# ooshyun/Speech-Enhancement-Pytorch

Measured on AMD Instinct MI355X. Metric: audio-sec/sec training, DCCRN 16kHz 2s bs32, higher is better.
Workload: dtype bf16; 1 GPU; DCCRN (kernel_num 16-32-64-128-256-256, complex LSTM 128, mask E) train step, 16 kHz 2-s clips, SI-SNR, Adam 3e-4, clip 5; per_gpu_batch=32, global_batch=32, samples_per_clip=32000, parallelism=dp1, launch=eager, inputs=resident in HBM

## Files before the change

### include/sehip.h

```cpp
#ifndef SEHIP_H
#define SEHIP_H
#include <stdint.h>

#ifdef __cplusplus
extern "C" {
#endif

const char* sehip_last_error(void);
const char* sehip_last_kernel(void);
int sehip_version(void);
int sehip_check_device(int device);

void* sehip_event_create(void);
int sehip_event_destroy(void* event);
int sehip_stream_depend(void* to_stream, void* from_stream, void* event);
int sehip_event_record(void* event, void* stream);
int sehip_stream_wait_event(void* stream, void* event);
void* sehip_stream_create(int priority_class);
int sehip_stream_destroy(void* stream);

int sehip_stft_frames(int n_samples, int win_len, int hop);
int sehip_stft_fwd(const float* wav , const float* window , int B, int N, int win_len, int hop,
                   int fft_len, float* spec , void* enc_in_bf16 , void* stream);
int sehip_istft_fwd(const float* spec, const float* mask , const float* window,
// ... 191 lines not shown
                           long rows, int Cr, float* gWrr, float* gWri, float* gWii, float* gBr, float* gBi, float* gslope,
                           float* bcoef , void* stream);
int sehip_cbn_bwd_finalize_n(const float* part, int nblk, const float* coef, const float* Wrr, const float* Wri, const float* Wii,
                             long rows, int Cr, float* gWrr, float* gWri, float* gWii, float* gBr, float* gBi, float* gslope,
                             float* bcoef , void* stream);
int sehip_cbn_bwd_fused(const void* dz, const void* dz2 , const void* y, const float* coef, const float* Wrr, const float* Wri,
                        const float* Wii, const float* slope, long rows, int Cr, int F, int Tst, int tfirst, float* rep, float* rep_next,
                        int nrep,
                        float* gWrr, float* gWri, float* gWii, float* gBr, float* gBi, float* gslope, void* dy, void* stream);
int sehip_cbn_bwd_reduce_fin(const void* dz, const void* dz2 , const void* y, const float* coef, const float* Wrr,
                             const float* Wri, const float* Wii, const float* slope, long rows, int Cr, int F, int Tst, int tfirst,
                             float* rep, int nrep, unsigned* ticket, float* gWrr, float* gWri, float* gWii, float* gBr, float* gBi,
                             float* gslope, float* bcoef , void* stream);
int sehip_cbn_bwd_apply(const void* dz, const void* dz2, const void* y, const float* coef, const float* bcoef,
                        const float* slope, long rows, int Cr, int F, int Tst, int tfirst, void* dy, void* stream);

long sehip_rbn_scratch_floats(long rows, int Cs);
int sehip_rbn_stats(const void* y, long rows, int Cs, int Cr, float* part, void* stream);
int sehip_rbn_finalize(const float* part, const float* w_re, const float* b_re, const float* w_im, const float* b_im, float* rm_re,
                       float* rv_re, float* rm_im, float* rv_im, long* nbt_re, long* nbt_im, long rows, int Cs, int Cr, float eps,
                       float momentum, int training, float* coef, void* stream);
int sehip_rbn_finalize_s(const float* part, const float* w_re, const float* b_re, const float* w_im, const float* b_im, float* rm_re,
                         float* rv_re, float* rm_im, float* rv_im, long* nbt_re, long* nbt_im, long rows, int Cs, int Cr, float eps,
                         float momentum, int training, const float* shift, float* coef, void* stream);
int sehip_rbn_apply(const void* y, const float* coef, long rows, int Cs, int Cr, void* z, void* stream);
int sehip_rbn_bwd_reduce(const void* dz, const void* y, const float* coef, long rows, int Cs, int Cr, float* part, void* stream);
int sehip_rbn_bwd_reduce_fin(const void* dz, const void* y, const float* coef, long rows, int Cs, int Cr, float* part, unsigned* ticket,
                             float* gw_re, float* gb_re, float* gw_im, float* gb_im, float* bcoef, void* stream);
int sehip_rbn_bwd_finalize(const float* part, const float* coef, long rows, int Cs, int Cr, float* gw_re, float* gb_re, float* gw_im,
                           float* gb_im, float* bcoef, void* stream);
// ... 213 lines not shown
```

### speech-enhancement-pytorch_amd/sehip/_lib.py

```python
import ctypes as C
import os

import torch

_HERE = os.path.dirname(os.path.abspath(__file__))
LIB_PATH = os.environ.get("SEHIP_LIB") or os.path.join(_HERE, "libsehip.so")


class SehipError(RuntimeError):
    pass


_lib = None

P = C.c_void_p
I = C.c_int
L = C.c_long
F = C.c_float
U = C.c_uint
D = C.c_double

_PROTOS = {
    "sehip_version": [],
    "sehip_check_device": [I],
# ... 79 lines not shown
    "sehip_unpack_grad_sums_perm": [P, P, P, L, P, P, I, P, P, P, P, P],
    "sehip_unpack_grad1": [P, P, L, P, P],
    "sehip_unpack_grad1_sums": [P, P, L, P, P, I, P, P, P, P, P],
    "sehip_unpack_grad_list_sums": [P, P, P, L, P, P, I, P, P, P],
    "sehip_unpack_grad_list": [P, P, P, L, P, P],
    "sehip_pack_bf16_runs": [P, P, P, L, P, P],
    "sehip_pack_bf16_runs_to": [P, P, P, P, L, P, P],
    "sehip_cbn_stats": [P, L, I, P, P],
    "sehip_cbn_finalize": [P, P, P, P, P, P, P, P, P, P, P, P, L, I, F, F, I, P, P],
    "sehip_cbn_finalize_n": [P, I, P, P, P, P, P, P, P, P, P, P, P, L, I, F, F, I, P, P],
    "sehip_cbn_apply": [P, P, P, L, I, P, P],
    "sehip_cbn_finalize_apply_n": [P, P, I, P, P, P, P, P, P, P, P, P, P, P, L, I, F, F, I, P, P, P, P],
    "sehip_cbn_bwd_reduce": [P, P, P, P, P, L, I, I, I, I, P, P],
    "sehip_cbn_bwd_finalize": [P, P, P, P, P, L, I, P, P, P, P, P, P, P, P],
    "sehip_cbn_bwd_apply": [P, P, P, P, P, P, L, I, I, I, I, P, P],
    "sehip_cbn_bwd_fused": [P, P, P, P, P, P, P, P, L, I, I, I, I, P, P, I, P, P, P, P, P, P, P, P],
    "sehip_cbn_bwd_reduce_fin": [P, P, P, P, P, P, P, P, L, I, I, I, I, P, I, P, P, P, P, P, P, P, P, P],
    "sehip_rbn_scratch_floats": [L, I],
    "sehip_rbn_stats": [P, L, I, I, P, P],
    "sehip_rbn_finalize": [P, P, P, P, P, P, P, P, P, P, P, L, I, I, F, F, I, P, P],
    "sehip_rbn_finalize_s": [P, P, P, P, P, P, P, P, P, P, P, L, I, I, F, F, I, P, P, P],
    "sehip_rbn_apply": [P, P, L, I, I, P, P],
    "sehip_rbn_bwd_reduce": [P, P, P, L, I, I, P, P],
    "sehip_rbn_bwd_reduce_fin": [P, P, P, L, I, I, P, P, P, P, P, P, P, P],
    "sehip_rbn_bwd_finalize": [P, P, L, I, I, P, P, P, P, P, P],
    "sehip_rbn_bwd_apply": [P, P, P, P, L, I, I, P, P],
    "sehip_dcunet_pack_input": [P, I, I, I, P, P],
    "sehip_dcunet_mask_fwd": [P, P, P, P, P, P, I, I, I, I, I, I, P, P, P],
    "sehip_dcunet_mask_bwd": [P, P, P, P, P, P, I, I, I, I, I, I, P, P, P],
    "sehip_dcunet_mask_fwd_bn": [P, P, P, P, P, P, P, I, I, I, I, I, I, P, P, P],
# ... 187 lines not shown
```

### speech-enhancement-pytorch_amd/sehip/csrc/cbn.hip

```cpp
#include <stdlib.h>
#include "common.h"

#define COEF_STRIDE 16


template <int CH> struct Raw;
template <> struct Raw<8> { typedef uint4 type; };
template <> struct Raw<4> { typedef uint2 type; };
template <int CH> struct Chunk { float v[CH]; };
__device__ __forceinline__ Chunk<8> unpack(uint4 u) {
    Chunk<8> c;
    c.v[0] = bf2f((bf16_raw)(u.x & 0xffff)); c.v[1] = bf2f((bf16_raw)(u.x >> 16));
    c.v[2] = bf2f((bf16_raw)(u.y & 0xffff)); c.v[3] = bf2f((bf16_raw)(u.y >> 16));
    c.v[4] = bf2f((bf16_raw)(u.z & 0xffff)); c.v[5] = bf2f((bf16_raw)(u.z >> 16));
    c.v[6] = bf2f((bf16_raw)(u.w & 0xffff)); c.v[7] = bf2f((bf16_raw)(u.w >> 16));
    return c;
}
__device__ __forceinline__ Chunk<4> unpack(uint2 u) {
    Chunk<4> c;
    c.v[0] = bf2f((bf16_raw)(u.x & 0xffff)); c.v[1] = bf2f((bf16_raw)(u.x >> 16));
    c.v[2] = bf2f((bf16_raw)(u.y & 0xffff)); c.v[3] = bf2f((bf16_raw)(u.y >> 16));
    return c;
}
__device__ __forceinline__ void pack_store(bf16_raw* p, const float (&v)[8]) {
// ... 138 lines not shown
        RVri[c] = rvri + momentum * (vri - rvri);
        RVii[c] = rvii + momentum * (vii * unb - rvii);
        if (c == 0 && nbt) nbt[0] += 1;
    } else {
        if (threadIdx.x != 0) return;
        mr = rmr; mi = rmi; vrr = rvrr; vri = rvri; vii = rvii;
    }
    float rec[15];
    cbn_fwd_record(mr, mi, vrr, vri, vii, eps, wrr, wri, wii, br_, bi_, rec);
    float* o = coef + (size_t)c * COEF_STRIDE;
#pragma unroll
    for (int i = 0; i < 15; ++i) o[i] = rec[i];
}

template <int CH>
__device__ __forceinline__ void stage_coef(const float* __restrict__ rec, int Cr, int nfield, float4* __restrict__ slot) {
    const int nq = Cr / CH;
    for (int i = threadIdx.x; i < Cr * nfield; i += 256) {
        const int c = i / nfield, f = i - c * nfield;
        slot[f * Cr + (c % CH) * nq + (c / CH)] = reinterpret_cast<const float4*>(rec)[c * (COEF_STRIDE / 4) + f];
    }
}

template <int U, int CH>
__global__ __launch_bounds__(256, 2) void cbn_apply_kernel(const bf16_raw* __restrict__ y, const float* __restrict__ coef,
                                                           const float* __restrict__ slope, long rows, int Cr,
                                                           bf16_raw* __restrict__ z) {
    typedef typename Raw<CH>::type raw_t;
    __shared__ float4 cl[2 * 256];
    const int nq = Cr / CH;
    const int C = 2 * Cr;
    const int q = threadIdx.x % nq, rl = threadIdx.x / nq, rpb = 256 / nq;
    const float a = slope[0];
    stage_coef<CH>(coef, Cr, 2, cl);
    __syncthreads();
// ... 140 lines not shown
    v.gi = *reinterpret_cast<const raw_t*>(dz + o + Cr);
    if (HAS2) {
        v.hr = *reinterpret_cast<const raw_t*>(dz2 + o);
        v.hi = *reinterpret_cast<const raw_t*>(dz2 + o + Cr);
    }
    return v;
}

struct CbnFin {
    const float *Wrr, *Wri, *Wii;
    float *gWrr, *gWri, *gWii, *gBr, *gBi, *gslope, *bcoef;
    unsigned* ticket;
};
__device__ __forceinline__ void cbn_bwd_record(float sdr, float sdi, float qrr, float qri, float qir, float qii, float urr, float uri,
                                               float uii, float vrr, float vri, float vii, float wrr, float wri, float wii, float n,
                                               float (&g5)[5], float (&o)[9], float real = 0.f);

template <int U, int CH, bool HAS2>
__global__ __launch_bounds__(256, 2) void cbn_bwd_reduce_kernel(const bf16_raw* __restrict__ dz, const bf16_raw* __restrict__ dz2,
                                                                const bf16_raw* __restrict__ y, const float* __restrict__ coef,
                                                                const float* __restrict__ slope, long rows, int Cr, int F,
                                                                int Tst, int tfirst, float* __restrict__ part, int nrep, const CbnFin fin) {
    __shared__ float lds[4 * 6 * 8 * 32];
    const int nq = Cr / CH;
    const int q = threadIdx.x % nq, rl = threadIdx.x / nq, rpb = 256 / nq;
    const int C = 2 * Cr;
    const float a = slope[0];
    float s[6][CH];
#pragma unroll
    for (int u = 0; u < 6; ++u)
#pragma unroll
        for (int j = 0; j < CH; ++j) s[u][j] = 0.f;
    float da = 0.f;
// ... 26 lines not shown
            s[0][j] += dr; s[1][j] += di;
            s[2][j] += dr * cr; s[3][j] += dr * ci; s[4][j] += di * cr; s[5][j] += di * ci;
        }
    };
    const long stride = (long)gridDim.x * rpb;
    long r = (long)blockIdx.x * rpb + rl;
    for (; r + (U - 1) * stride < rows; r += U * stride) {
        RowIn<CH, HAS2> v[U];
#pragma unroll
        for (int u = 0; u < U; ++u) v[u] = load_row<CH, HAS2>(y, dz, dz2, (r + u * stride) * C + q * CH, Cr);
#pragma unroll
        for (int u = 0; u < U; ++u) row(v[u], r + u * stride);
    }
    if (U > 1)
        for (; r < rows; r += stride) row(load_row<CH, HAS2>(y, dz, dz2, r * C + q * CH, Cr), r);
    block_partials<6, CH>(s, nq, Cr, part, 6 * Cr + 1, lds, nrep);
    da = wave_sum(da);
    __syncthreads();
    if ((threadIdx.x & 63) == 0) lds[threadIdx.x >> 6] = da;
    __syncthreads();
    if (threadIdx.x == 0) {
        const float t = lds[0] + lds[1] + lds[2] + lds[3];
        if (nrep > 0) atomicAdd(&part[(size_t)(blockIdx.x % nrep) * (6 * Cr + 1) + 6 * Cr], t);
        else part[(size_t)blockIdx.x * (6 * Cr + 1) + 6 * Cr] = t;
    }
    if (nrep <= 0 || fin.ticket == nullptr) return;
    asm volatile("s_waitcnt vmcnt(0)" ::: "memory");
    __syncthreads();
    __shared__ unsigned is_last;
    if (threadIdx.x == 0) {
        __builtin_amdgcn_fence(__ATOMIC_RELEASE, "agent");
        asm volatile("s_waitcnt vmcnt(0)" ::: "memory");
        is_last = __hip_atomic_fetch_add(fin.ticket, 1u, __ATOMIC_RELAXED, __HIP_MEMORY_SCOPE_AGENT) == gridDim.x - 1 ? 1u : 0u;
    }
    __syncthreads();
    if (!is_last) return;
    if (threadIdx.x == 0) {
        __builtin_amdgcn_fence(__ATOMIC_ACQUIRE, "agent");
        asm volatile("s_waitcnt vmcnt(0)" ::: "memory");
    }
    __syncthreads();
    const int st = 6 * Cr + 1;
    for (int c = threadIdx.x; c < Cr; c += 256) {
        const float* k = coef + (size_t)c * COEF_STRIDE;
        const float urr = k[8], uri = k[9], uii = k[10], vrr = k[11], vri = k[12], vii = k[13];
        const float wrr = fin.Wrr[c], wri = fin.Wri[c], wii = fin.Wii[c];
        double a6[6] = {0.0, 0.0, 0.0, 0.0, 0.0, 0.0};
        for (int r0 = 0; r0 < nrep; r0 += 8) {
            float v[8][6];
#pragma unroll
            for (int r = 0; r < 8; ++r)
#pragma unroll
                for (int kk = 0; kk < 6; ++kk) v[r][kk] = part[(size_t)(r0 + r < nrep ? r0 + r : 0) * st + kk * Cr + c];
#pragma unroll
            for (int r = 0; r < 8; ++r)
#pragma unroll
                for (int kk = 0; kk < 6; ++kk) a6[kk] += r0 + r < nrep ? (double)v[r][kk] : 0.0;
        }
        float g5[5], rec[9];
        cbn_bwd_record((float)a6[0], (float)a6[1], (float)a6[2], (float)a6[3], (float)a6[4], (float)a6[5], urr, uri, uii, vrr, vri, vii,
                       wrr, wri, wii, (float)rows, g5, rec, k[14]);
        fin.gWrr[c] = g5[0]; fin.gWri[c] = g5[1]; fin.gWii[c] = g5[2]; fin.gBr[c] = g5[3]; fin.gBi[c] = g5[4];
        float* o = fin.bcoef + (size_t)c * COEF_STRIDE;
#pragma unroll
        for (int i = 0; i < 9; ++i) o[i] = rec[i];
    }
    if (threadIdx.x == 255) {
        double ds = 0.0;
        for (int r = 0; r < nrep; ++r) ds += (double)part[(size_t)r * st + 6 * Cr];
        fin.gslope[0] = (float)ds;
    }
    __syncthreads();
    for (int i = threadIdx.x; i < nrep * st; i += 256) part[i] = 0.f;
    if (threadIdx.x == 0) __hip_atomic_store(fin.ticket, 0u, __ATOMIC_RELAXED, __HIP_MEMORY_SCOPE_AGENT);
}

__device__ __forceinline__ void cbn_bwd_record(float sdr, float sdi, float qrr, float qri, float qir, float qii, float urr, float uri,
                                               float uii, float vrr, float vri, float vii, float wrr, float wri, float wii, float n,
                                               float (&g5)[5], float (&o)[9], float real) {
    if (real != 0.f) wri = 0.f;
    const float prr = qrr * urr + qri * uri, pri = qrr * uri + qri * uii;
    const float pir = qir * urr + qii * uri, pii = qir * uri + qii * uii;
    g5[0] = prr; g5[1] = pri + pir; g5[2] = pii; g5[3] = sdr; g5[4] = sdi;
    const float hrr = wrr * qrr + wri * qir, hri = wrr * qri + wri * qii;
    const float hir = wri * qrr + wii * qir, hii = wri * qri + wii * qii;
    const float dUrr = hrr, dUri = hri + hir, dUii = hii;
    const float tau = vrr + vii;
    const float delta = vrr * vii - vri * vri;
    const float s = sqrtf(delta);
    const float t = sqrtf(tau + 2.f * s);
    const float rst = 1.f / (s * t);
    const float d_rst = dUrr * (s + vii) - dUri * vri + dUii * (s + vrr);
    float d_s = (dUrr + dUii) * rst;
    float d_vii = dUrr * rst, d_vrr = dUii * rst, d_vri = -dUri * rst;
    d_s += d_rst * (-rst / s);
    const float d_t = d_rst * (-rst / t);
    const float d_tau = d_t / (2.f * t);
    d_s += d_t / t;
    const float d_delta = d_s / (2.f * s);
    d_vrr += d_delta * vii + d_tau;
    d_vii += d_delta * vrr + d_tau;
    d_vri += d_delta * (-2.f * vri);
    const float arr = urr * wrr + uri * wri, ari = urr * wri + uri * wii;
    const float air = uri * wrr + uii * wri, aii = uri * wri + uii * wii;
    o[0] = arr; o[1] = ari; o[2] = air; o[3] = aii;
    o[4] = 2.f * d_vrr / n; o[5] = d_vri / n; o[6] = 2.f * d_vii / n;
    o[7] = -(arr * sdr + ari * sdi) / n;
    o[8] = -(air * sdr + aii * sdi) / n;
    if (real != 0.f) { o[5] = 0.f; g5[1] = 0.f; }
}

template <int MAXB>
__global__ void cbn_bwd_finalize_kernel(const float* __restrict__ part, int nblk, const float* __restrict__ coef,
                                        const float* __restrict__ Wrr, const float* __restrict__ Wri,
                                        const float* __restrict__ Wii, long rows, int Cr, float* __restrict__ gWrr,
                                        float* __restrict__ gWri, float* __restrict__ gWii, float* __restrict__ gBr,
                                        float* __restrict__ gBi, float* __restrict__ gslope, float* __restrict__ bcoef) {
    const int c = blockIdx.x;
    const int st = 6 * Cr + 1;
    if (c == Cr) {
        double ds[1];
        wave_reduce_partials<1, MAXB>(part, nblk, st, 6 * Cr, Cr, ds);
        if (threadIdx.x == 0) gslope[0] = (float)ds[0];
        return;
    }
    const float* k = coef + (size_t)c * COEF_STRIDE;
    const float urr = k[8], uri = k[9], uii = k[10], vrr = k[11], vri = k[12], vii = k[13];
    const float wrr = Wrr[c], wri = Wri[c], wii = Wii[c];
    double a[6];
    wave_reduce_partials<6, MAXB>(part, nblk, st, c, Cr, a);
    const float sdr = (float)a[0], sdi = (float)a[1], qrr = (float)a[2], qri = (float)a[3], qir = (float)a[4], qii = (float)a[5];
    if (threadIdx.x != 0) return;
    float g5[5], rec[9];
    cbn_bwd_record(sdr, sdi, qrr, qri, qir, qii, urr, uri, uii, vrr, vri, vii, wrr, wri, wii, (float)rows, g5, rec, k[14]);
    gWrr[c] = g5[0]; gWri[c] = g5[1]; gWii[c] = g5[2]; gBr[c] = g5[3]; gBi[c] = g5[4];
    float* o = bcoef + (size_t)c * COEF_STRIDE;
#pragma unroll
    for (int i = 0; i < 9; ++i) o[i] = rec[i];
}

template <int U, int CH, bool HAS2>
__global__ __launch_bounds__(256, 2) void cbn_bwd_apply_kernel(const bf16_raw* __restrict__ dz, const bf16_raw* __restrict__ dz2,
                                                               const bf16_raw* __restrict__ y, const float* __restrict__ coef,
                                                               const float* __restrict__ bcoef, const float* __restrict__ slope,
                                                               long rows, int Cr, int F, int Tst, int tfirst,
                                                               bf16_raw* __restrict__ dy) {
    __shared__ float4 cl[5 * 256];
    const int nq = Cr / CH;
    const int C = 2 * Cr;
    const int q = threadIdx.x % nq, rl = threadIdx.x / nq, rpb = 256 / nq;
    const float a = slope[0];
    stage_coef<CH>(coef, Cr, 2, cl);
    stage_coef<CH>(bcoef, Cr, 3, cl + 2 * Cr);
    __syncthreads();
    float4 zc[CH], mb[CH], A[CH], E[CH];
    float ki[CH];
#pragma unroll
    for (int j = 0; j < CH; ++j) {
        zc[j] = cl[j * nq + q];
        mb[j] = cl[Cr + j * nq + q];
        A[j] = cl[2 * Cr + j * nq + q];
        E[j] = cl[3 * Cr + j * nq + q];
        ki[j] = cl[4 * Cr + j * nq + q].x;
    }
    auto row = [&](const RowIn<CH, HAS2>& v, long r) {
        const bool dropped = tfirst > 0 && (int)(((unsigned)r / (unsigned)F) % (unsigned)Tst) < tfirst;
        const Chunk<CH> xr = unpack(v.yr), xi = unpack(v.yi);
        Chunk<CH> gr = unpack(v.gr), gi = unpack(v.gi);
        if (HAS2) {
            const Chunk<CH> hr = unpack(v.hr), hi = unpack(v.hi);
#pragma unroll
            for (int j = 0; j < CH; ++j) { gr.v[j] += hr.v[j]; gi.v[j] += hi.v[j]; }
        }
        float orr[CH], oii[CH];
#pragma unroll
        for (int j = 0; j < CH; ++j) {
            const float cr = xr.v[j] - mb[j].x, ci = xi.v[j] - mb[j].y;
            const float vr = zc[j].x * cr + zc[j].y * ci + mb[j].z;
            const float vi = zc[j].z * cr + zc[j].w * ci + mb[j].w;
            float dr = dropped ? 0.f : gr.v[j], di = dropped ? 0.f : gi.v[j];
            if (!(vr > 0.f)) dr *= a;
            if (!(vi > 0.f)) di *= a;
            orr[j] = A[j].x * dr + A[j].y * di + E[j].x * cr + E[j].y * ci + E[j].w;
            oii[j] = A[j].z * dr + A[j].w * di + E[j].y * cr + E[j].z * ci + ki[j];
        }
        pack_store(dy + r * C + q * CH, orr);
        pack_store(dy + r * C + Cr + q * CH, oii);
    };
    const long stride = (long)gridDim.x * rpb;
    long r = (long)blockIdx.x * rpb + rl;
    for (; r + (U - 1) * stride < rows; r += U * stride) {
        RowIn<CH, HAS2> v[U];
#pragma unroll
        for (int u = 0; u < U; ++u) v[u] = load_row<CH, HAS2>(y, dz, dz2, (r + u * stride) * C + q * CH, Cr);
#pragma unroll
        for (int u = 0; u < U; ++u) row(v[u], r + u * stride);
    }
    if (U > 1)
        for (; r < rows; r += stride) row(load_row<CH, HAS2>(y, dz, dz2, r * C + q * CH, Cr), r);
}

template <int U, int CH, bool HAS2>
__global__ __launch_bounds__(256, 2) void cbn_bwd_apply_fin_kernel(const bf16_raw* __restrict__ dz, const bf16_raw* __restrict__ dz2,
                                                               const bf16_raw* __restrict__ y, const float* __restrict__ coef,
                                                               const float* __restrict__ rep , int nrep,
                                                               float* __restrict__ rep_next ,
                                                               const float* __restrict__ Wrr, const float* __restrict__ Wri,
                                                               const float* __restrict__ Wii, float* __restrict__ gWrr,
                                                               float* __restrict__ gWri, float* __restrict__ gWii, float* __restrict__ gBr,
                                                               float* __restrict__ gBi, float* __restrict__ gslope,
                                                               const float* __restrict__ slope, long rows, int Cr, int F, int Tst,
                                                               int tfirst, bf16_raw* __restrict__ dy, int dbg_mode) {
    __shared__ float4 cl[5 * 256];
    const int nq = Cr / CH;
    const int C = 2 * Cr;
    const int q = threadIdx.x % nq, rl = threadIdx.x / nq, rpb = 256 / nq;
    const float a = slope[0];
    for (int i = blockIdx.x * 256 + threadIdx.x; i < nrep * (6 * Cr + 1); i += gridDim.x * 256) rep_next[i] = 0.f;
    stage_coef<CH>(coef, Cr, 2, cl);
    for (int c = threadIdx.x; c < Cr; c += 256) {
        const float* k = coef + (size_t)c * COEF_STRIDE;
        auto ldg = [&](const float* p_) { return (dbg_mode & 2) ? __hip_atomic_load(p_, __ATOMIC_RELAXED, __HIP_MEMORY_SCOPE_AGENT) : *p_; };
        const float urr = ldg(k + 8), uri = ldg(k + 9), uii = ldg(k + 10), vrr = ldg(k + 11), vri = ldg(k + 12), vii = ldg(k + 13);
        const float wrr = ldg(Wrr + c), wri = ldg(Wri + c), wii = ldg(Wii + c);
        double a6[6] = {0.0, 0.0, 0.0, 0.0, 0.0, 0.0};
        for (int r0 = 0; r0 < nrep; r0 += 8) {
            float v[8][6];
#pragma unroll
            for (int r = 0; r < 8; ++r)
#pragma unroll
                for (int kk = 0; kk < 6; ++kk) {
                    const float* pr = &rep[(size_t)(r0 + r < nrep ? r0 + r : 0) * (6 * Cr + 1) + kk * Cr + c];
                    v[r][kk] = (dbg_mode & 1) ? __hip_atomic_load(pr, __ATOMIC_RELAXED, __HIP_MEMORY_SCOPE_AGENT) : *pr;
                }
#pragma unroll
            for (int r = 0; r < 8; ++r)
#pragma unroll
                for (int kk = 0; kk < 6; ++kk) a6[kk] += r0 + r < nrep ? (double)v[r][kk] : 0.0;
        }
        float g5[5], rec[9];
        cbn_bwd_record((float)a6[0], (float)a6[1], (float)a6[2], (float)a6[3], (float)a6[4], (float)a6[5], urr, uri, uii, vrr, vri, vii,
                       wrr, wri, wii, (float)rows, g5, rec, k[14]);
        const int slot = (c % CH) * nq + (c / CH);
        cl[2 * Cr + slot] = make_float4(rec[0], rec[1], rec[2], rec[3]);
        cl[3 * Cr + slot] = make_float4(rec[4], rec[5], rec[6], rec[7]);
        cl[4 * Cr + slot] = make_float4(rec[8], 0.f, 0.f, 0.f);
        if (blockIdx.x == 0) { gWrr[c] = g5[0]; gWri[c] = g5[1]; gWii[c] = g5[2]; gBr[c] = g5[3]; gBi[c] = g5[4]; }
    }
    if (blockIdx.x == 0 && threadIdx.x == 255) {
        double ds = 0.0;
        for (int r = 0; r < nrep; ++r) ds += (double)rep[(size_t)r * (6 * Cr + 1) + 6 * Cr];
        gslope[0] = (float)ds;
    }
    __syncthreads();
    float4 zc[CH], mb[CH], A[CH], E[CH];
    float ki[CH];
#pragma unroll
    for (int j = 0; j < CH; ++j) {
        zc[j] = cl[j * nq + q];
        mb[j] = cl[Cr + j * nq + q];
        A[j] = cl[2 * Cr + j * nq + q];
        E[j] = cl[3 * Cr + j * nq + q];
        ki[j] = cl[4 * Cr + j * nq + q].x;
    }
    auto row = [&](const RowIn<CH, HAS2>& v, long r) {
        const bool dropped = tfirst > 0 && (int)(((unsigned)r / (unsigned)F) % (unsigned)Tst) < tfirst;
        const Chunk<CH> xr = unpack(v.yr), xi = unpack(v.yi);
        Chunk<CH> gr = unpack(v.gr), gi = unpack(v.gi);
        if (HAS2) {
            const Chunk<CH> hr = unpack(v.hr), hi = unpack(v.hi);
#pragma unroll
            for (int j = 0; j < CH; ++j) { gr.v[j] += hr.v[j]; gi.v[j] += hi.v[j]; }
        }
        float orr[CH], oii[CH];
#pragma unroll
        for (int j = 0; j < CH; ++j) {
            const float cr = xr.v[j] - mb[j].x, ci = xi.v[j] - mb[j].y;
            const float vr = zc[j].x * cr + zc[j].y * ci + mb[j].z;
            const float vi = zc[j].z * cr + zc[j].w * ci + mb[j].w;
            float dr = dropped ? 0.f : gr.v[j], di = dropped ? 0.f : gi.v[j];
            if (!(vr > 0.f)) dr *= a;
            if (!(vi > 0.f)) di *= a;
            orr[j] = A[j].x * dr + A[j].y * di + E[j].x * cr + E[j].y * ci + E[j].w;
            oii[j] = A[j].z * dr + A[j].w * di + E[j].y * cr + E[j].z * ci + ki[j];
        }
        pack_store(dy + r * C + q * CH, orr);
        pack_store(dy + r * C + Cr + q * CH, oii);
    };
    const long stride = (long)gridDim.x * rpb;
    long r = (long)blockIdx.x * rpb + rl;
    for (; r + (U - 1) * stride < rows; r += U * stride) {
        RowIn<CH, HAS2> v[U];
#pragma unroll
        for (int u = 0; u < U; ++u) v[u] = load_row<CH, HAS2>(y, dz, dz2, (r + u * stride) * C + q * CH, Cr);
#pragma unroll
        for (int u = 0; u < U; ++u) row(v[u], r + u * stride);
    }
    if (U > 1)
        for (; r < rows; r += stride) row(load_row<CH, HAS2>(y, dz, dz2, r * C + q * CH, Cr), r);
}

static int check_cbn(const char* who, long rows, int Cr) {
    SEHIP_REQUIRE(rows > 0, "%s: empty input", who);
    SEHIP_REQUIRE(Cr >= 8 && Cr <= 256 && (Cr & (Cr - 1)) == 0,
                  "%s: complex channels Cr=%d must be a power of two in [8, 256]", who, Cr);
    return 0;
}
static int grid_for(long work_items) {
    long g = (work_items + 255) / 256;
    if (g > 4096) g = 4096;
    if (g < 1) g = 1;
    return (int)g;
}

// ... 103 lines not shown
        case 4 * 16 + 8: CBN_FAPP(4, 8); break;
        case 1 * 16 + 4: CBN_FAPP(1, 4); break;
        case 4 * 16 + 4: CBN_FAPP(4, 4); break;
        default: CBN_FAPP(2, 4); break;
    }
#undef CBN_FAPP
    SEHIP_CHECK_LAUNCH("cbn_finalize_apply_n");
    return 0;
}

static int cbn_bwd_reduce_launch(const void* dz, const void* dz2, const void* y, const float* coef, const float* slope,
                                 long rows, int Cr, int F, int Tst, int tfirst, float* part, int nrep, void* stream,
                                 const CbnFin fin = CbnFin{}) {
    if (int e = check_cbn("cbn_bwd_reduce", rows, Cr)) return e;
    SEHIP_REQUIRE(rows < (1L << 31), "cbn_bwd_reduce: %ld rows exceed the 32-bit frame arithmetic", rows);
#define CBN_RED(U, CH, H2) cbn_bwd_reduce_kernel<U, CH, H2><<<stat_blocks(rows, Cr), 256, 0, (hipStream_t)stream>>>( \
        (const bf16_raw*)dz, (const bf16_raw*)dz2, (const bf16_raw*)y, coef, slope, rows, Cr, F, Tst, tfirst, part, nrep, fin)
#define CBN_RED2(U, CH) do { if (dz2) CBN_RED(U, CH, true); else CBN_RED(U, CH, false); } while (0)
    switch (unroll_rows_bwd() * 16 + cbn_ch(Cr)) {
        case 1 * 16 + 8: CBN_RED2(1, 8); break;
        case 2 * 16 + 8: CBN_RED2(2, 8); break;
        case 4 * 16 + 8: CBN_RED2(4, 8); break;
        case 1 * 16 + 4: CBN_RED2(1, 4); break;
        case 4 * 16 + 4: CBN_RED2(4, 4); break;
        default: CBN_RED2(2, 4); break;
    }
#undef CBN_RED2
#undef CBN_RED
    SEHIP_CHECK_LAUNCH("cbn_bwd_reduce");
    return 0;
}
extern "C" int sehip_cbn_bwd_reduce(const void* dz, const void* dz2, const void* y, const float* coef, const float* slope,
                                    long rows, int Cr, int F, int Tst, int tfirst, float* part, void* stream) {
    return cbn_bwd_reduce_launch(dz, dz2, y, coef, slope, rows, Cr, F, Tst, tfirst, part, 0, stream);
}

extern "C" int sehip_cbn_bwd_reduce_fin(const void* dz, const void* dz2, const void* y, const float* coef, const float* Wrr,
                                        const float* Wri, const float* Wii, const float* slope, long rows, int Cr, int F, int Tst,
                                        int tfirst, float* rep, int nrep, unsigned* ticket, float* gWrr, float* gWri, float* gWii,
                                        float* gBr, float* gBi, float* gslope, float* bcoef, void* stream) {
    SEHIP_REQUIRE(nrep >= 1 && nrep <= 64 && rep && ticket && bcoef, "cbn_bwd_reduce_fin: %d rows of sums (1..64), rows / ticket / bcoef", nrep);
    SEHIP_REQUIRE(!sehip_deterministic(), "cbn_bwd_reduce_fin: not part of the deterministic schedule (fp32 atomics): use "
// ... 15 lines not shown
extern "C" int sehip_cbn_bwd_finalize_n(const float* part, int nblk, const float* coef, const float* Wrr, const float* Wri,
                                        const float* Wii, long rows, int Cr, float* gWrr, float* gWri, float* gWii, float* gBr,
                                        float* gBi, float* gslope, float* bcoef, void* stream) {
    if (int e = check_cbn("cbn_bwd_finalize_n", rows, Cr)) return e;
    SEHIP_REQUIRE(nblk >= 1 && nblk <= 1024, "cbn_bwd_finalize_n: %d rows of sums (1..1024)", nblk);
    if (nblk <= CBN_MAX_BLOCKS)
        cbn_bwd_finalize_kernel<CBN_MAX_BLOCKS><<<Cr + 1, 64, 0, (hipStream_t)stream>>>(part, nblk, coef, Wrr, Wri, Wii, rows, Cr, gWrr, gWri,
                                                                                    gWii, gBr, gBi, gslope, bcoef);
    else
        cbn_bwd_finalize_kernel<1024><<<Cr + 1, 64, 0, (hipStream_t)stream>>>(part, nblk, coef, Wrr, Wri, Wii, rows, Cr, gWrr, gWri, gWii, gBr,
                                                                          gBi, gslope, bcoef);
    SEHIP_CHECK_LAUNCH("cbn_bwd_finalize_n");
    return 0;
}

extern "C" int sehip_cbn_bwd_apply(const void* dz, const void* dz2, const void* y, const float* coef, const float* bcoef,
                                   const float* slope, long rows, int Cr, int F, int Tst, int tfirst, void* dy, void* stream) {
    if (int e = check_cbn("cbn_bwd_apply", rows, Cr)) return e;
    SEHIP_REQUIRE(rows < (1L << 31), "cbn_bwd_apply: %ld rows exceed the 32-bit frame arithmetic", rows);
#define CBN_BAPP(U, CH, H2) cbn_bwd_apply_kernel<U, CH, H2><<<apply_blocks(rows, Cr, true), 256, 0, (hipStream_t)stream>>>( \
        (const bf16_raw*)dz, (const bf16_raw*)dz2, (const bf16_raw*)y, coef, bcoef, slope, rows, Cr, F, Tst, tfirst, (bf16_raw*)dy)
#define CBN_BAPP2(U, CH) do { if (dz2) CBN_BAPP(U, CH, true); else CBN_BAPP(U, CH, false); } while (0)
    switch (unroll_rows_bwd() * 16 + cbn_ch(Cr)) {
        case 1 * 16 + 8: CBN_BAPP2(1, 8); break;
        case 2 * 16 + 8: CBN_BAPP2(2, 8); break;
        case 4 * 16 + 8: CBN_BAPP2(4, 8); break;
        case 1 * 16 + 4: CBN_BAPP2(1, 4); break;
        case 4 * 16 + 4: CBN_BAPP2(4, 4); break;
        default: CBN_BAPP2(2, 4); break;
    }
#undef CBN_BAPP2
#undef CBN_BAPP
    SEHIP_CHECK_LAUNCH("cbn_bwd_apply");
    return 0;
}

extern "C" int sehip_cbn_bwd_fused(const void* dz, const void* dz2, const void* y, const float* coef, const float* Wrr, const float* Wri,
                                   const float* Wii, const float* slope, long rows, int Cr, int F, int Tst, int tfirst, float* rep,
                                   float* rep_next, int nrep, float* gWrr, float* gWri, float* gWii, float* gBr, float* gBi, float* gslope, void* dy, void* stream) {
    if (int e = check_cbn("cbn_bwd_fused", rows, Cr)) return e;
    SEHIP_REQUIRE(rows < (1L << 31), "cbn_bwd_fused: %ld rows exceed the 32-bit frame arithmetic", rows);
    SEHIP_REQUIRE(nrep >= 1 && nrep <= 64 && rep != nullptr && rep_next != nullptr && rep_next != rep,
                  "cbn_bwd_fused: %d rows of sums (1..64), two distinct sets", nrep);
    if (int e = cbn_bwd_reduce_launch(dz, dz2, y, coef, slope, rows, Cr, F, Tst, tfirst, rep, nrep, stream)) return e;
    static const int dbg_mode = env_int("SEHIP_BWD_FIN_DBG", 0);
#define CBN_BFIN(U, CH, H2) cbn_bwd_apply_fin_kernel<U, CH, H2><<<apply_blocks(rows, Cr), 256, 0, (hipStream_t)stream>>>(              \
// ... 17 lines not shown
```

Before: 19910 audio-s/s.

## Streamline complex BN backward apply with packed math, 32-bit offsets and fewer coefs

Moves the complex batch-norm backward apply loop into a shared helper that uses two-wide float vector math, 32-bit byte offsets when the tensor is small enough, and a compile-time branch for the dropped-frame check. It reuses the forward whitening coefficients instead of recomputing them, which shrinks staged LDS coefficients from five to four slots per channel. It also templates the reduce kernel on whether the finalize tail exists, so that code is compiled out when unused. The aims are lower register pressure, less address arithmetic and less LDS traffic in a bandwidth-bound elementwise pass, at the cost of more template instantiations and reliance on the stored z fields matching the old recomputed values.

```diff
diff --git a/include/sehip.h b/include/sehip.h
--- a/include/sehip.h
+++ b/include/sehip.h
@@ -229,6 +229,7 @@
                              float* gslope, float* bcoef , void* stream);
 int sehip_cbn_bwd_apply(const void* dz, const void* dz2, const void* y, const float* coef, const float* bcoef,
                         const float* slope, long rows, int Cr, int F, int Tst, int tfirst, void* dy, void* stream);
+int sehip_cbn_bwd_apply_offsets32(long rows, int Cr);
 
 long sehip_rbn_scratch_floats(long rows, int Cs);
 int sehip_rbn_stats(const void* y, long rows, int Cs, int Cr, float* part, void* stream);
diff --git a/speech-enhancement-pytorch_amd/sehip/_lib.py b/speech-enhancement-pytorch_amd/sehip/_lib.py
--- a/speech-enhancement-pytorch_amd/sehip/_lib.py
+++ b/speech-enhancement-pytorch_amd/sehip/_lib.py
@@ -117,6 +117,7 @@
     "sehip_cbn_bwd_reduce": [P, P, P, P, P, L, I, I, I, I, P, P],
     "sehip_cbn_bwd_finalize": [P, P, P, P, P, L, I, P, P, P, P, P, P, P, P],
     "sehip_cbn_bwd_apply": [P, P, P, P, P, P, L, I, I, I, I, P, P],
+    "sehip_cbn_bwd_apply_offsets32": [L, I],
     "sehip_cbn_bwd_fused": [P, P, P, P, P, P, P, P, L, I, I, I, I, P, P, I, P, P, P, P, P, P, P, P],
     "sehip_cbn_bwd_reduce_fin": [P, P, P, P, P, P, P, P, L, I, I, I, I, P, I, P, P, P, P, P, P, P, P, P],
     "sehip_rbn_scratch_floats": [L, I],
diff --git a/speech-enhancement-pytorch_amd/sehip/csrc/cbn.hip b/speech-enhancement-pytorch_amd/sehip/csrc/cbn.hip
--- a/speech-enhancement-pytorch_amd/sehip/csrc/cbn.hip
+++ b/speech-enhancement-pytorch_amd/sehip/csrc/cbn.hip
@@ -1,4 +1,5 @@
 #include <stdlib.h>
+#include <type_traits>
 #include "common.h"
 
 #define COEF_STRIDE 16
@@ -8,6 +9,7 @@
 template <> struct Raw<8> { typedef uint4 type; };
 template <> struct Raw<4> { typedef uint2 type; };
 template <int CH> struct Chunk { float v[CH]; };
+typedef float f2 __attribute__((ext_vector_type(2)));
 __device__ __forceinline__ Chunk<8> unpack(uint4 u) {
     Chunk<8> c;
     c.v[0] = bf2f((bf16_raw)(u.x & 0xffff)); c.v[1] = bf2f((bf16_raw)(u.x >> 16));
@@ -176,11 +178,11 @@
 }
 
 template <int CH>
-__device__ __forceinline__ void stage_coef(const float* __restrict__ rec, int Cr, int nfield, float4* __restrict__ slot) {
+__device__ __forceinline__ void stage_coef(const float* __restrict__ rec, int Cr, int nfield, float4* __restrict__ slot, int field0 = 0) {
     const int nq = Cr / CH;
     for (int i = threadIdx.x; i < Cr * nfield; i += 256) {
         const int c = i / nfield, f = i - c * nfield;
-        slot[f * Cr + (c % CH) * nq + (c / CH)] = reinterpret_cast<const float4*>(rec)[c * (COEF_STRIDE / 4) + f];
+        slot[f * Cr + (c % CH) * nq + (c / CH)] = reinterpret_cast<const float4*>(rec)[c * (COEF_STRIDE / 4) + field0 + f];
     }
 }
 
@@ -351,9 +353,9 @@
 };
 __device__ __forceinline__ void cbn_bwd_record(float sdr, float sdi, float qrr, float qri, float qir, float qii, float urr, float uri,
                                                float uii, float vrr, float vri, float vii, float wrr, float wri, float wii, float n,
-                                               float (&g5)[5], float (&o)[9], float real = 0.f);
-
-template <int U, int CH, bool HAS2>
+                                               const float4 z, float (&g5)[5], float (&o)[9], float real = 0.f);
+
+template <int U, int CH, bool HAS2, bool FIN>
 __global__ __launch_bounds__(256, 2) void cbn_bwd_reduce_kernel(const bf16_raw* __restrict__ dz, const bf16_raw* __restrict__ dz2,
                                                                 const bf16_raw* __restrict__ y, const float* __restrict__ coef,
                                                                 const float* __restrict__ slope, long rows, int Cr, int F,
@@ -410,6 +412,7 @@
     }
     if (U > 1)
         for (; r < rows; r += stride) row(load_row<CH, HAS2>(y, dz, dz2, r * C + q * CH, Cr), r);
+    if (!FIN) nrep = 0;
     block_partials<6, CH>(s, nq, Cr, part, 6 * Cr + 1, lds, nrep);
     da = wave_sum(da);
     __syncthreads();
@@ -420,7 +423,7 @@
         if (nrep > 0) atomicAdd(&part[(size_t)(blockIdx.x % nrep) * (6 * Cr + 1) + 6 * Cr], t);
         else part[(size_t)blockIdx.x * (6 * Cr + 1) + 6 * Cr] = t;
     }
-    if (nrep <= 0 || fin.ticket == nullptr) return;
+    if (!FIN || nrep <= 0 || fin.ticket == nullptr) return;
     asm volatile("s_waitcnt vmcnt(0)" ::: "memory");
     __syncthreads();
     __shared__ unsigned is_last;
@@ -440,6 +443,7 @@
     for (int c = threadIdx.x; c < Cr; c += 256) {
         const float* k = coef + (size_t)c * COEF_STRIDE;
         const float urr = k[8], uri = k[9], uii = k[10], vrr = k[11], vri = k[12], vii = k[13];
+        const float4 zf = *reinterpret_cast<const float4*>(k);
         const float wrr = fin.Wrr[c], wri = fin.Wri[c], wii = fin.Wii[c];
         double a6[6] = {0.0, 0.0, 0.0, 0.0, 0.0, 0.0};
         for (int r0 = 0; r0 < nrep; r0 += 8) {
@@ -455,7 +459,7 @@
         }
         float g5[5], rec[9];
         cbn_bwd_record((float)a6[0], (float)a6[1], (float)a6[2], (float)a6[3], (float)a6[4], (float)a6[5], urr, uri, uii, vrr, vri, vii,
-                       wrr, wri, wii, (float)rows, g5, rec, k[14]);
+                       wrr, wri, wii, (float)rows, zf, g5, rec, k[14]);
         fin.gWrr[c] = g5[0]; fin.gWri[c] = g5[1]; fin.gWii[c] = g5[2]; fin.gBr[c] = g5[3]; fin.gBi[c] = g5[4];
         float* o = fin.bcoef + (size_t)c * COEF_STRIDE;
 #pragma unroll
@@ -473,7 +477,7 @@
 
 __device__ __forceinline__ void cbn_bwd_record(float sdr, float sdi, float qrr, float qri, float qir, float qii, float urr, float uri,
                                                float uii, float vrr, float vri, float vii, float wrr, float wri, float wii, float n,
-                                               float (&g5)[5], float (&o)[9], float real) {
+                                               const float4 z, float (&g5)[5], float (&o)[9], float real) {
     if (real != 0.f) wri = 0.f;
     const float prr = qrr * urr + qri * uri, pri = qrr * uri + qri * uii;
     const float pir = qir * urr + qii * uri, pii = qir * uri + qii * uii;
@@ -497,8 +501,7 @@
     d_vrr += d_delta * vii + d_tau;
     d_vii += d_delta * vrr + d_tau;
     d_vri += d_delta * (-2.f * vri);
-    const float arr = urr * wrr + uri * wri, ari = urr * wri + uri * wii;
-    const float air = uri * wrr + uii * wri, aii = uri * wri + uii * wii;
+    const float arr = z.x, ari = z.z, air = z.y, aii = z.w;
     o[0] = arr; o[1] = ari; o[2] = air; o[3] = aii;
     o[4] = 2.f * d_vrr / n; o[5] = d_vri / n; o[6] = 2.f * d_vii / n;
     o[7] = -(arr * sdr + ari * sdi) / n;
@@ -522,78 +525,114 @@
     }
     const float* k = coef + (size_t)c * COEF_STRIDE;
     const float urr = k[8], uri = k[9], uii = k[10], vrr = k[11], vri = k[12], vii = k[13];
+    const float4 zf = *reinterpret_cast<const float4*>(k);
     const float wrr = Wrr[c], wri = Wri[c], wii = Wii[c];
     double a[6];
     wave_reduce_partials<6, MAXB>(part, nblk, st, c, Cr, a);
     const float sdr = (float)a[0], sdi = (float)a[1], qrr = (float)a[2], qri = (float)a[3], qir = (float)a[4], qii = (float)a[5];
     if (threadIdx.x != 0) return;
     float g5[5], rec[9];
-    cbn_bwd_record(sdr, sdi, qrr, qri, qir, qii, urr, uri, uii, vrr, vri, vii, wrr, wri, wii, (float)rows, g5, rec, k[14]);
+    cbn_bwd_record(sdr, sdi, qrr, qri, qir, qii, urr, uri, uii, vrr, vri, vii, wrr, wri, wii, (float)rows, zf, g5, rec, k[14]);
     gWrr[c] = g5[0]; gWri[c] = g5[1]; gWii[c] = g5[2]; gBr[c] = g5[3]; gBi[c] = g5[4];
     float* o = bcoef + (size_t)c * COEF_STRIDE;
 #pragma unroll
     for (int i = 0; i < 9; ++i) o[i] = rec[i];
 }
 
-template <int U, int CH, bool HAS2>
+template <int U, int CH, bool HAS2, bool O32, bool DROP>
+__device__ __forceinline__ void cbn_bwd_apply_rows(const bf16_raw* __restrict__ dz, const bf16_raw* __restrict__ dz2,
+                                                   const bf16_raw* __restrict__ y, const float4* __restrict__ cl, float a, long rows,
+                                                   int Cr, int F, int Tst, int tfirst, bf16_raw* __restrict__ dy) {
+    typedef typename Raw<CH>::type raw_t;
+    typedef typename std::conditional<O32, unsigned, size_t>::type off_t;
+    const int lq = __builtin_ctz((unsigned)(Cr / CH)), nq = 1 << lq;
+    const int q = threadIdx.x & (nq - 1), rl = threadIdx.x >> lq, rpb = 256 >> lq;
+    f2 zx[CH / 2], zy[CH / 2], zz[CH / 2], zw[CH / 2], mx[CH / 2], my[CH / 2], bx[CH / 2], by[CH / 2];
+    f2 err[CH / 2], eri[CH / 2], eii[CH / 2], kr[CH / 2], ki[CH / 2];
+#pragma unroll
+    for (int p = 0; p < CH / 2; ++p) {
+        const float4 z0 = cl[(2 * p) * nq + q], z1 = cl[(2 * p + 1) * nq + q];
+        const float4 m0 = cl[Cr + (2 * p) * nq + q], m1 = cl[Cr + (2 * p + 1) * nq + q];
+        const float4 e0 = cl[2 * Cr + (2 * p) * nq + q], e1 = cl[2 * Cr + (2 * p + 1) * nq + q];
+        zx[p] = f2{z0.x, z1.x}; zy[p] = f2{z0.y, z1.y}; zz[p] = f2{z0.z, z1.z}; zw[p] = f2{z0.w, z1.w};
+        mx[p] = f2{m0.x, m1.x}; my[p] = f2{m0.y, m1.y}; bx[p] = f2{m0.z, m1.z}; by[p] = f2{m0.w, m1.w};
+        err[p] = f2{e0.x, e1.x}; eri[p] = f2{e0.y, e1.y}; eii[p] = f2{e0.z, e1.z}; kr[p] = f2{e0.w, e1.w};
+        ki[p] = f2{cl[3 * Cr + (2 * p) * nq + q].x, cl[3 * Cr + (2 * p + 1) * nq + q].x};
+    }
+    const char* yi = reinterpret_cast<const char*>(y + Cr);
+    const char* gi = reinterpret_cast<const char*>(dz + Cr);
+    const char* hi = reinterpret_cast<const char*>(dz2 + Cr);
+    char* oi = reinterpret_cast<char*>(dy + Cr);
+    auto load = [&](off_t o) {
+        RowIn<CH, HAS2> v;
+        v.yr = *reinterpret_cast<const raw_t*>(reinterpret_cast<const char*>(y) + o);
+        v.yi = *reinterpret_cast<const raw_t*>(yi + o);
+        v.gr = *reinterpret_cast<const raw_t*>(reinterpret_cast<const char*>(dz) + o);
+        v.gi = *reinterpret_cast<const raw_t*>(gi + o);
+        if (HAS2) {
+            v.hr = *reinterpret_cast<const raw_t*>(reinterpret_cast<const char*>(dz2) + o);
+            v.hi = *reinterpret_cast<const raw_t*>(hi + o);
+        }
+        return v;
+    };
+    auto row = [&](const RowIn<CH, HAS2>& v, unsigned r, off_t o) {
+        const bool dropped = DROP && (int)((r / (unsigned)F) % (unsigned)Tst) < tfirst;
+        const Chunk<CH> xr = unpack(v.yr), xi = unpack(v.yi);
+        Chunk<CH> gr = unpack(v.gr), gi = unpack(v.gi);
+        if (HAS2) {
+            const Chunk<CH> hr = unpack(v.hr), hi = unpack(v.hi);
+#pragma unroll
+            for (int j = 0; j < CH; ++j) { gr.v[j] += hr.v[j]; gi.v[j] += hi.v[j]; }
+        }
+        float orr[CH], oii[CH];
+#pragma unroll
+        for (int p = 0; p < CH / 2; ++p) {
+            const int j = 2 * p;
+            const f2 cr = f2{xr.v[j], xr.v[j + 1]} - mx[p], ci = f2{xi.v[j], xi.v[j + 1]} - my[p];
+            const f2 vr = zx[p] * cr + zy[p] * ci + bx[p];
+            const f2 vi = zz[p] * cr + zw[p] * ci + by[p];
+            f2 dr = dropped ? f2{0.f, 0.f} : f2{gr.v[j], gr.v[j + 1]}, di = dropped ? f2{0.f, 0.f} : f2{gi.v[j], gi.v[j + 1]};
+            const f2 ar = dr * a, ai = di * a;
+            if (!(vr.x > 0.f)) dr.x = ar.x;
+            if (!(vr.y > 0.f)) dr.y = ar.y;
+            if (!(vi.x > 0.f)) di.x = ai.x;
+            if (!(vi.y > 0.f)) di.y = ai.y;
+            const f2 pr = zx[p] * dr + zz[p] * di + err[p] * cr + eri[p] * ci + kr[p];
+            const f2 pi = zy[p] * dr + zw[p] * di + eri[p] * cr + eii[p] * ci + ki[p];
+            orr[j] = pr.x; orr[j + 1] = pr.y; oii[j] = pi.x; oii[j + 1] = pi.y;
+        }
+        pack_store(reinterpret_cast<bf16_raw*>(reinterpret_cast<char*>(dy) + o), orr);
+        pack_store(reinterpret_cast<bf16_raw*>(oi + o), oii);
+    };
+    const unsigned nrow = (unsigned)rows, stride = gridDim.x * rpb;
+    const off_t rowb = (off_t)(4 * Cr), strb = (off_t)stride * rowb;
+    unsigned r = blockIdx.x * rpb + rl;
+    off_t o = (off_t)r * rowb + (off_t)(q * CH * 2);
+#pragma unroll 1
+    for (; r + (U - 1) * stride < nrow; r += U * stride, o += U * strb) {
+        RowIn<CH, HAS2> v[U];
+#pragma unroll
+        for (int u = 0; u < U; ++u) v[u] = load(o + u * strb);
+#pragma unroll
+        for (int u = 0; u < U; ++u) row(v[u], r + u * stride, o + u * strb);
+    }
+    if (U > 1)
+        for (; r < nrow; r += stride, o += strb) row(load(o), r, o);
+}
+
+template <int U, int CH, bool HAS2, bool O32>
 __global__ __launch_bounds__(256, 2) void cbn_bwd_apply_kernel(const bf16_raw* __restrict__ dz, const bf16_raw* __restrict__ dz2,
                                                                const bf16_raw* __restrict__ y, const float* __restrict__ coef,
                                                                const float* __restrict__ bcoef, const float* __restrict__ slope,
                                                                long rows, int Cr, int F, int Tst, int tfirst,
                                                                bf16_raw* __restrict__ dy) {
-    __shared__ float4 cl[5 * 256];
-    const int nq = Cr / CH;
-    const int C = 2 * Cr;
-    const int q = threadIdx.x % nq, rl = threadIdx.x / nq, rpb = 256 / nq;
+    __shared__ float4 cl[4 * 256];
     const float a = slope[0];
     stage_coef<CH>(coef, Cr, 2, cl);
-    stage_coef<CH>(bcoef, Cr, 3, cl + 2 * Cr);
-    __syncthreads();
-    float4 zc[CH], mb[CH], A[CH], E[CH];
-    float ki[CH];
-#pragma unroll
-    for (int j = 0; j < CH; ++j) {
-        zc[j] = cl[j * nq + q];
-        mb[j] = cl[Cr + j * nq + q];
-        A[j] = cl[2 * Cr + j * nq + q];
-        E[j] = cl[3 * Cr + j * nq + q];
-        ki[j] = cl[4 * Cr + j * nq + q].x;
-    }
-    auto row = [&](const RowIn<CH, HAS2>& v, long r) {
-        const bool dropped = tfirst > 0 && (int)(((unsigned)r / (unsigned)F) % (unsigned)Tst) < tfirst;
-        const Chunk<CH> xr = unpack(v.yr), xi = unpack(v.yi);
-        Chunk<CH> gr = unpack(v.gr), gi = unpack(v.gi);
-        if (HAS2) {
-            const Chunk<CH> hr = unpack(v.hr), hi = unpack(v.hi);
-#pragma unroll
-            for (int j = 0; j < CH; ++j) { gr.v[j] += hr.v[j]; gi.v[j] += hi.v[j]; }
-        }
-        float orr[CH], oii[CH];
-#pragma unroll
-        for (int j = 0; j < CH; ++j) {
-            const float cr = xr.v[j] - mb[j].x, ci = xi.v[j] - mb[j].y;
-            const float vr = zc[j].x * cr + zc[j].y * ci + mb[j].z;
-            const float vi = zc[j].z * cr + zc[j].w * ci + mb[j].w;
-            float dr = dropped ? 0.f : gr.v[j], di = dropped ? 0.f : gi.v[j];
-            if (!(vr > 0.f)) dr *= a;
-            if (!(vi > 0.f)) di *= a;
-            orr[j] = A[j].x * dr + A[j].y * di + E[j].x * cr + E[j].y * ci + E[j].w;
-            oii[j] = A[j].z * dr + A[j].w * di + E[j].y * cr + E[j].z * ci + ki[j];
-        }
-        pack_store(dy + r * C + q * CH, orr);
-        pack_store(dy + r * C + Cr + q * CH, oii);
-    };
-    const long stride = (long)gridDim.x * rpb;
-    long r = (long)blockIdx.x * rpb + rl;
-    for (; r + (U - 1) * stride < rows; r += U * stride) {
-        RowIn<CH, HAS2> v[U];
-#pragma unroll
-        for (int u = 0; u < U; ++u) v[u] = load_row<CH, HAS2>(y, dz, dz2, (r + u * stride) * C + q * CH, Cr);
-#pragma unroll
-        for (int u = 0; u < U; ++u) row(v[u], r + u * stride);
-    }
-    if (U > 1)
-        for (; r < rows; r += stride) row(load_row<CH, HAS2>(y, dz, dz2, r * C + q * CH, Cr), r);
+    stage_coef<CH>(bcoef, Cr, 2, cl + 2 * Cr, 1);
+    __syncthreads();
+    if (tfirst > 0) cbn_bwd_apply_rows<U, CH, HAS2, O32, true>(dz, dz2, y, cl, a, rows, Cr, F, Tst, tfirst, dy);
+    else cbn_bwd_apply_rows<U, CH, HAS2, O32, false>(dz, dz2, y, cl, a, rows, Cr, F, Tst, tfirst, dy);
 }
 
 template <int U, int CH, bool HAS2>
@@ -607,10 +646,8 @@
                                                                float* __restrict__ gBi, float* __restrict__ gslope,
                                                                const float* __restrict__ slope, long rows, int Cr, int F, int Tst,
                                                                int tfirst, bf16_raw* __restrict__ dy, int dbg_mode) {
-    __shared__ float4 cl[5 * 256];
+    __shared__ float4 cl[4 * 256];
     const int nq = Cr / CH;
-    const int C = 2 * Cr;
-    const int q = threadIdx.x % nq, rl = threadIdx.x / nq, rpb = 256 / nq;
     const float a = slope[0];
     for (int i = blockIdx.x * 256 + threadIdx.x; i < nrep * (6 * Cr + 1); i += gridDim.x * 256) rep_next[i] = 0.f;
     stage_coef<CH>(coef, Cr, 2, cl);
@@ -619,6 +656,7 @@
         auto ldg = [&](const float* p_) { return (dbg_mode & 2) ? __hip_atomic_load(p_, __ATOMIC_RELAXED, __HIP_MEMORY_SCOPE_AGENT) : *p_; };
         const float urr = ldg(k + 8), uri = ldg(k + 9), uii = ldg(k + 10), vrr = ldg(k + 11), vri = ldg(k + 12), vii = ldg(k + 13);
         const float wrr = ldg(Wrr + c), wri = ldg(Wri + c), wii = ldg(Wii + c);
+        const float4 zf = *reinterpret_cast<const float4*>(k);
         double a6[6] = {0.0, 0.0, 0.0, 0.0, 0.0, 0.0};
         for (int r0 = 0; r0 < nrep; r0 += 8) {
             float v[8][6];
@@ -636,11 +674,10 @@
         }
         float g5[5], rec[9];
         cbn_bwd_record((float)a6[0], (float)a6[1], (float)a6[2], (float)a6[3], (float)a6[4], (float)a6[5], urr, uri, uii, vrr, vri, vii,
-                       wrr, wri, wii, (float)rows, g5, rec, k[14]);
+                       wrr, wri, wii, (float)rows, zf, g5, rec, k[14]);
         const int slot = (c % CH) * nq + (c / CH);
-        cl[2 * Cr + slot] = make_float4(rec[0], rec[1], rec[2], rec[3]);
-        cl[3 * Cr + slot] = make_float4(rec[4], rec[5], rec[6], rec[7]);
-        cl[4 * Cr + slot] = make_float4(rec[8], 0.f, 0.f, 0.f);
+        cl[2 * Cr + slot] = make_float4(rec[4], rec[5], rec[6], rec[7]);
+        cl[3 * Cr + slot] = make_float4(rec[8], 0.f, 0.f, 0.f);
         if (blockIdx.x == 0) { gWrr[c] = g5[0]; gWri[c] = g5[1]; gWii[c] = g5[2]; gBr[c] = g5[3]; gBi[c] = g5[4]; }
     }
     if (blockIdx.x == 0 && threadIdx.x == 255) {
@@ -649,51 +686,8 @@
         gslope[0] = (float)ds;
     }
     __syncthreads();
-    float4 zc[CH], mb[CH], A[CH], E[CH];
-    float ki[CH];
-#pragma unroll
-    for (int j = 0; j < CH; ++j) {
-        zc[j] = cl[j * nq + q];
-        mb[j] = cl[Cr + j * nq + q];
-        A[j] = cl[2 * Cr + j * nq + q];
-        E[j] = cl[3 * Cr + j * nq + q];
-        ki[j] = cl[4 * Cr + j * nq + q].x;
-    }
-    auto row = [&](const RowIn<CH, HAS2>& v, long r) {
-        const bool dropped = tfirst > 0 && (int)(((unsigned)r / (unsigned)F) % (unsigned)Tst) < tfirst;
-        const Chunk<CH> xr = unpack(v.yr), xi = unpack(v.yi);
-        Chunk<CH> gr = unpack(v.gr), gi = unpack(v.gi);
-        if (HAS2) {
-            const Chunk<CH> hr = unpack(v.hr), hi = unpack(v.hi);
-#pragma unroll
-            for (int j = 0; j < CH; ++j) { gr.v[j] += hr.v[j]; gi.v[j] += hi.v[j]; }
-        }
-        float orr[CH], oii[CH];
-#pragma unroll
-        for (int j = 0; j < CH; ++j) {
-            const float cr = xr.v[j] - mb[j].x, ci = xi.v[j] - mb[j].y;
-            const float vr = zc[j].x * cr + zc[j].y * ci + mb[j].z;
-            const float vi = zc[j].z * cr + zc[j].w * ci + mb[j].w;
-            float dr = dropped ? 0.f : gr.v[j], di = dropped ? 0.f : gi.v[j];
-            if (!(vr > 0.f)) dr *= a;
-            if (!(vi > 0.f)) di *= a;
-            orr[j] = A[j].x * dr + A[j].y * di + E[j].x * cr + E[j].y * ci + E[j].w;
-            oii[j] = A[j].z * dr + A[j].w * di + E[j].y * cr + E[j].z * ci + ki[j];
-        }
-        pack_store(dy + r * C + q * CH, orr);
-        pack_store(dy + r * C + Cr + q * CH, oii);
-    };
-    const long stride = (long)gridDim.x * rpb;
-    long r = (long)blockIdx.x * rpb + rl;
-    for (; r + (U - 1) * stride < rows; r += U * stride) {
-        RowIn<CH, HAS2> v[U];
-#pragma unroll
-        for (int u = 0; u < U; ++u) v[u] = load_row<CH, HAS2>(y, dz, dz2, (r + u * stride) * C + q * CH, Cr);
-#pragma unroll
-        for (int u = 0; u < U; ++u) row(v[u], r + u * stride);
-    }
-    if (U > 1)
-        for (; r < rows; r += stride) row(load_row<CH, HAS2>(y, dz, dz2, r * C + q * CH, Cr), r);
+    if (tfirst > 0) cbn_bwd_apply_rows<U, CH, HAS2, false, true>(dz, dz2, y, cl, a, rows, Cr, F, Tst, tfirst, dy);
+    else cbn_bwd_apply_rows<U, CH, HAS2, false, false>(dz, dz2, y, cl, a, rows, Cr, F, Tst, tfirst, dy);
 }
 
 static int check_cbn(const char* who, long rows, int Cr) {
@@ -827,9 +821,10 @@
                                  const CbnFin fin = CbnFin{}) {
     if (int e = check_cbn("cbn_bwd_reduce", rows, Cr)) return e;
     SEHIP_REQUIRE(rows < (1L << 31), "cbn_bwd_reduce: %ld rows exceed the 32-bit frame arithmetic", rows);
-#define CBN_RED(U, CH, H2) cbn_bwd_reduce_kernel<U, CH, H2><<<stat_blocks(rows, Cr), 256, 0, (hipStream_t)stream>>>( \
+#define CBN_RED(U, CH, H2, FIN) cbn_bwd_reduce_kernel<U, CH, H2, FIN><<<stat_blocks(rows, Cr), 256, 0, (hipStream_t)stream>>>( \
         (const bf16_raw*)dz, (const bf16_raw*)dz2, (const bf16_raw*)y, coef, slope, rows, Cr, F, Tst, tfirst, part, nrep, fin)
-#define CBN_RED2(U, CH) do { if (dz2) CBN_RED(U, CH, true); else CBN_RED(U, CH, false); } while (0)
+#define CBN_RED1(U, CH, H2) do { if (nrep > 0) CBN_RED(U, CH, H2, true); else CBN_RED(U, CH, H2, false); } while (0)
+#define CBN_RED2(U, CH) do { if (dz2) CBN_RED1(U, CH, true); else CBN_RED1(U, CH, false); } while (0)
     switch (unroll_rows_bwd() * 16 + cbn_ch(Cr)) {
         case 1 * 16 + 8: CBN_RED2(1, 8); break;
         case 2 * 16 + 8: CBN_RED2(2, 8); break;
@@ -839,6 +834,7 @@
         default: CBN_RED2(2, 4); break;
     }
 #undef CBN_RED2
+#undef CBN_RED1
 #undef CBN_RED
     SEHIP_CHECK_LAUNCH("cbn_bwd_reduce");
     return 0;
@@ -884,13 +880,17 @@
     return 0;
 }
 
+extern "C" int sehip_cbn_bwd_apply_offsets32(long rows, int Cr) { return rows > 0 && Cr > 0 && rows < (1L << 31) / (2L * Cr) ? 1 : 0; }
+
 extern "C" int sehip_cbn_bwd_apply(const void* dz, const void* dz2, const void* y, const float* coef, const float* bcoef,
                                    const float* slope, long rows, int Cr, int F, int Tst, int tfirst, void* dy, void* stream) {
     if (int e = check_cbn("cbn_bwd_apply", rows, Cr)) return e;
     SEHIP_REQUIRE(rows < (1L << 31), "cbn_bwd_apply: %ld rows exceed the 32-bit frame arithmetic", rows);
-#define CBN_BAPP(U, CH, H2) cbn_bwd_apply_kernel<U, CH, H2><<<apply_blocks(rows, Cr, true), 256, 0, (hipStream_t)stream>>>( \
+    const bool o32 = sehip_cbn_bwd_apply_offsets32(rows, Cr) != 0;
+#define CBN_BAPP(U, CH, H2, O32) cbn_bwd_apply_kernel<U, CH, H2, O32><<<apply_blocks(rows, Cr, true), 256, 0, (hipStream_t)stream>>>( \
         (const bf16_raw*)dz, (const bf16_raw*)dz2, (const bf16_raw*)y, coef, bcoef, slope, rows, Cr, F, Tst, tfirst, (bf16_raw*)dy)
-#define CBN_BAPP2(U, CH) do { if (dz2) CBN_BAPP(U, CH, true); else CBN_BAPP(U, CH, false); } while (0)
+#define CBN_BAPP1(U, CH, H2) do { if (o32) CBN_BAPP(U, CH, H2, true); else CBN_BAPP(U, CH, H2, false); } while (0)
+#define CBN_BAPP2(U, CH) do { if (dz2) CBN_BAPP1(U, CH, true); else CBN_BAPP1(U, CH, false); } while (0)
     switch (unroll_rows_bwd() * 16 + cbn_ch(Cr)) {
         case 1 * 16 + 8: CBN_BAPP2(1, 8); break;
         case 2 * 16 + 8: CBN_BAPP2(2, 8); break;
@@ -900,6 +900,7 @@
         default: CBN_BAPP2(2, 4); break;
     }
 #undef CBN_BAPP2
+#undef CBN_BAPP1
 #undef CBN_BAPP
     SEHIP_CHECK_LAUNCH("cbn_bwd_apply");
     return 0;
```

Result: no change. 19880 audio-s/s (-0.2%).
